# tokamak-network/Tokamak-zk-EVM

Hardware: AMD Instinct MI355X
Metric: constraints/sec (prove step) (higher is better)
Workload: dtype u32 limbs (255-bit Fr / 381-bit Fq modular integer arithmetic)

## Files before the change

include/tkmk.h:

```cpp
#ifndef TKMK_H
#define TKMK_H
#include <stdbool.h>
#include <stddef.h>
#include <stdint.h>

#ifdef __cplusplus
extern "C" {
#endif

typedef enum {
    TKMK_SUCCESS = 0,
    TKMK_ERR_INVALID_DEVICE = 1,
    TKMK_ERR_OUT_OF_MEMORY = 2,
    TKMK_ERR_INVALID_POINTER = 3,
    TKMK_ERR_ALLOCATION_FAILED = 4,
    TKMK_ERR_DEALLOCATION_FAILED = 5,
    TKMK_ERR_COPY_FAILED = 6,
    TKMK_ERR_SYNCHRONIZATION_FAILED = 7,
    TKMK_ERR_STREAM_CREATION_FAILED = 8,
    TKMK_ERR_STREAM_DESTRUCTION_FAILED = 9,
    TKMK_ERR_API_NOT_IMPLEMENTED = 10,
    TKMK_ERR_INVALID_ARGUMENT = 11,
    TKMK_ERR_NO_DEVICE = 12,
    TKMK_ERR_UNKNOWN = 999
// ... 270 lines not shown
tkmk_error bls12_381_polynomial_degree(const tkmk_polynomial *p, int64_t *degree);
tkmk_error bls12_381_polynomial_copy_coeffs(const tkmk_polynomial *p, size_t start, size_t count, tkmk_fr *out, bool out_on_device);
tkmk_error bls12_381_polynomial_get_coeff(const tkmk_polynomial *p, size_t idx, tkmk_fr *out_host);
tkmk_error bls12_381_polynomial_coeffs_device_ptr(tkmk_polynomial *p, tkmk_fr **ptr, size_t *n);
tkmk_error bls12_381_polynomial_evaluate(const tkmk_polynomial *p, const tkmk_fr *x_host, tkmk_fr *out_host);
tkmk_error bls12_381_polynomial_add(const tkmk_polynomial *a, const tkmk_polynomial *b, tkmk_polynomial **out);
tkmk_error bls12_381_polynomial_subtract(const tkmk_polynomial *a, const tkmk_polynomial *b, tkmk_polynomial **out);
tkmk_error bls12_381_polynomial_multiply(const tkmk_polynomial *a, const tkmk_polynomial *b, tkmk_polynomial **out);
tkmk_error bls12_381_polynomial_multiply_by_scalar(const tkmk_polynomial *a, const tkmk_fr *s_host, tkmk_polynomial **out);
tkmk_error bls12_381_polynomial_slice(const tkmk_polynomial *p, size_t offset, size_t stride, size_t size, tkmk_polynomial **out);
tkmk_error bls12_381_polynomial_divide(const tkmk_polynomial *num, const tkmk_polynomial *den, tkmk_polynomial **quot, tkmk_polynomial **rem);

tkmk_error tkmk_r1cs_eval_rows(const uint32_t *row_ptr_dev, const uint32_t *wire_dev, const tkmk_fr *coeff_dev, uint32_t n_rows,
                               uint32_t nnz, const tkmk_fr *variables_dev, uint32_t n_wires, uint32_t n_placements,
                               const uint32_t *out_slot_dev, uint32_t n, tkmk_fr *out_dev, tkmk_stream stream);

typedef struct tkmk_r1cs_library tkmk_r1cs_library;
tkmk_error tkmk_r1cs_library_create(uint32_t n_sub, const uint32_t *n_rows, const uint32_t *n_wires, const uint32_t *const *row_ptr,
                                    const uint32_t *const *wire, const tkmk_fr *const *coeff, tkmk_r1cs_library **out);
tkmk_error tkmk_r1cs_library_destroy(tkmk_r1cs_library *lib);
tkmk_error tkmk_r1cs_library_eval(const tkmk_r1cs_library *lib, const tkmk_fr *vars_dev, const uint32_t *placement_id_dev,
                                  const uint64_t *placement_var_offset_dev, uint32_t n_placements, uint32_t n, uint32_t s_max,
                                  tkmk_fr *u_dev, tkmk_fr *v_dev, tkmk_fr *w_dev, tkmk_stream stream);
tkmk_error tkmk_r1cs_library_mix(const tkmk_r1cs_library *lib, const tkmk_fr *const *weight_dev, const uint8_t *const *col_dev, uint32_t n,
                                 uint32_t n_cols, uint32_t out_stride, tkmk_fr *u_dev, tkmk_fr *v_dev, tkmk_fr *w_dev, tkmk_stream stream);
tkmk_error tkmk_fr_outer(const tkmk_fr *col_dev, uint32_t rows, const tkmk_fr *row_dev, uint32_t cols, uint32_t out_stride, tkmk_fr *out_dev,
                         tkmk_stream stream);
tkmk_error tkmk_witness_route(const tkmk_fr *vars_dev, const uint64_t *var_offset_dev, const uint32_t *slot_dev, uint32_t n_placements,
                              const uint32_t *list_wire_dev, const uint32_t *list_row_dev, uint32_t n_list, tkmk_fr *matrix_dev,
                              uint32_t matrix_stride, tkmk_fr *scalars_out_dev, uint32_t *index_out_dev, uint32_t index_inner,
                              int index_add_slot, tkmk_stream stream);
tkmk_error tkmk_fr_scatter_table(const tkmk_fr *table_dev, uint64_t table_len, const uint32_t *src_idx_dev, const uint32_t *dst_idx_dev,
                                 uint64_t n, tkmk_fr *out_dev, uint64_t out_len, tkmk_stream stream);
tkmk_error tkmk_witness_check_r1cs(const tkmk_fr *u_dev, const tkmk_fr *v_dev, const tkmk_fr *w_dev, uint32_t n_rows, uint32_t n_cols,
                                   uint32_t stride, uint32_t *bad_count_dev, uint32_t *first_bad_row_dev, uint64_t *total_bad_out,
                                   tkmk_stream stream);
tkmk_error tkmk_witness_check_copy(const tkmk_fr *b_dev, uint32_t rows, uint32_t cols, uint32_t stride, const uint32_t *dst_idx_dev,
                                   const uint32_t *src_x_dev, const uint32_t *src_y_dev, uint64_t n_entries, uint64_t *bad_entries_out,
                                   uint64_t *first_bad_entry_out, tkmk_stream stream);
tkmk_error tkmk_witness_check_copy_split(const tkmk_fr *b_local_dev, uint64_t local_cells, const uint32_t *dst_local_dev,
                                         const tkmk_fr *sources_dev, uint64_t n_sources, const uint32_t *src_slot_dev, uint64_t n,
                                         uint64_t *bad_entries_out, uint64_t *first_bad_entry_out, tkmk_stream stream);
tkmk_error tkmk_host_malloc(void **ptr, size_t bytes);
tkmk_error tkmk_host_free(void *ptr);

tkmk_error tkmk_msm_set_pipeline_streams(int n);
// ... 17 lines not shown
```

tokamak-zk-evm_amd/csrc/witness.hip:

```cpp
#include <mutex>
#include <vector>

#include "common.h"
#include "r1cs_library.h"

__global__ __launch_bounds__(256) void k_r1cs_library_eval(const uint32_t *__restrict__ rowptr, const uint32_t *__restrict__ wire,
                                                          const fr_t *__restrict__ coeff_mont, const uint32_t *__restrict__ desc,
                                                          const fr_t *__restrict__ vars, const uint32_t *__restrict__ pl_id,
                                                          const uint64_t *__restrict__ pl_off, uint32_t s_max, fr_t *__restrict__ u,
                                                          fr_t *__restrict__ v, fr_t *__restrict__ w) {
    const uint32_t p = blockIdx.z, m = blockIdx.y;
    const uint32_t row = blockIdx.x * blockDim.x + threadIdx.x;
    const uint32_t *d = desc + 8 * pl_id[p];
    if (row >= d[6]) return;
    const uint32_t *rp = rowptr + d[m];
    const uint32_t eb = d[3 + m];
    const fr_t *x = vars + pl_off[p];
    fr_t acc = Fr::zero();
    for (uint32_t k = rp[row]; k < rp[row + 1]; k++)
        acc = Fr::add(acc, Fr::mul(Fr::canon(tk_load(x + wire[eb + k])), tk_load(coeff_mont + eb + k)));
    fr_t *out = m == 0 ? u : m == 1 ? v : w;
    tk_store(out + (uint64_t)row * s_max + p, acc);
}
__global__ __launch_bounds__(256) void k_fr_to_mont(const fr_t *__restrict__ in, fr_t *__restrict__ out, uint64_t n) {
    uint64_t i = (uint64_t)blockIdx.x * blockDim.x + threadIdx.x;
    if (i < n) tk_store(out + i, Fr::to_mont(Fr::canon(tk_load(in + i))));
}

TK_API tkmk_error tkmk_r1cs_library_create(uint32_t n_sub, const uint32_t *n_rows, const uint32_t *n_wires, const uint32_t *const *row_ptr,
                                           const uint32_t *const *wire, const tkmk_fr *const *coeff, tkmk_r1cs_library **out) {
    if (!out || !n_rows || !n_wires || !row_ptr || !wire || !coeff) return TKMK_ERR_INVALID_POINTER;
    TK_TRY(tk_require_device());
    std::vector<uint32_t> rp_all, wire_all, desc(8 * (size_t)n_sub);
    std::vector<tkmk_fr> coeff_all;
// ... 38 lines not shown
    if (e == TKMK_SUCCESS) e = up((void **)&lib->d_coeff, coeff_all.data(), coeff_all.size() * sizeof(tkmk_fr));
    if (e == TKMK_SUCCESS) e = up((void **)&lib->d_desc, desc.data(), desc.size() * 4);
    if (e == TKMK_SUCCESS) {
        hipLaunchKernelGGL(k_fr_to_mont, tk_div_up(coeff_all.size(), 256), 256, 0, 0, (const fr_t *)lib->d_coeff, lib->d_coeff,
                           (uint64_t)coeff_all.size());
        if (hipGetLastError() != hipSuccess || hipDeviceSynchronize() != hipSuccess) e = TKMK_ERR_UNKNOWN;
    }
    if (e != TKMK_SUCCESS) {
        (void)hipFree(lib->d_rowptr), (void)hipFree(lib->d_wire), (void)hipFree(lib->d_coeff), (void)hipFree(lib->d_desc);
        delete lib;
        return e;
    }
    *out = lib;
    return TKMK_SUCCESS;
}
TK_API tkmk_error tkmk_r1cs_library_destroy(tkmk_r1cs_library *lib) {
    if (!lib) return TKMK_SUCCESS;
    (void)hipDeviceSynchronize();
    (void)hipFree(lib->d_rowptr), (void)hipFree(lib->d_wire), (void)hipFree(lib->d_coeff), (void)hipFree(lib->d_desc);
    delete lib;
    return TKMK_SUCCESS;
}

TK_API tkmk_error tkmk_r1cs_library_eval(const tkmk_r1cs_library *lib, const tkmk_fr *vars_dev, const uint32_t *placement_id_dev,
                                         const uint64_t *placement_var_offset_dev, uint32_t n_placements, uint32_t n, uint32_t s_max,
                                         tkmk_fr *u_dev, tkmk_fr *v_dev, tkmk_fr *w_dev, tkmk_stream stream) {
    if (!lib || !u_dev || !v_dev || !w_dev) return TKMK_ERR_INVALID_POINTER;
    if (n_placements && (!vars_dev || !placement_id_dev || !placement_var_offset_dev)) return TKMK_ERR_INVALID_POINTER;
    if (n_placements > s_max || lib->max_rows > n) return TKMK_ERR_INVALID_ARGUMENT;
    TK_TRY(tk_require_device());
    hipStream_t s = tk_stream(stream);
    const size_t bytes = (size_t)n * s_max * sizeof(fr_t);
    TK_HIP(hipMemsetAsync(u_dev, 0, bytes, s));
    TK_HIP(hipMemsetAsync(v_dev, 0, bytes, s));
    TK_HIP(hipMemsetAsync(w_dev, 0, bytes, s));
    if (n_placements && lib->max_rows) {
        hipLaunchKernelGGL(k_r1cs_library_eval, dim3(tk_div_up(lib->max_rows, 256), 3, n_placements), 256, 0, s, lib->d_rowptr, lib->d_wire,
                           (const fr_t *)lib->d_coeff, lib->d_desc, (const fr_t *)vars_dev, placement_id_dev, placement_var_offset_dev,
                           s_max, (fr_t *)u_dev, (fr_t *)v_dev, (fr_t *)w_dev);
        TK_HIP(hipGetLastError());
    }
    return TKMK_SUCCESS;
}

__global__ __launch_bounds__(256) void k_witness_route(const fr_t *__restrict__ vars, const uint64_t *__restrict__ var_off,
                                                      const uint32_t *__restrict__ slot, uint32_t n_placements,
                                                      const uint32_t *__restrict__ list_wire, const uint32_t *__restrict__ list_row,
                                                      uint32_t n_list, fr_t *__restrict__ matrix, uint32_t matrix_stride,
                                                      fr_t *__restrict__ scalars_out, uint32_t *__restrict__ index_out, uint32_t index_inner,
                                                      int index_add_slot) {
    uint64_t g = (uint64_t)blockIdx.x * blockDim.x + threadIdx.x;
    if (g >= (uint64_t)n_placements * n_list) return;
    uint32_t i = (uint32_t)(g / n_list), e = (uint32_t)(g - (uint64_t)i * n_list);
    fr_t val = tk_load(vars + var_off[i] + list_wire[e]);
    const uint32_t row = list_row[e], sl = slot[i];
    if (matrix) tk_store(matrix + (uint64_t)row * matrix_stride + sl, val);
    if (scalars_out) {
        tk_store(scalars_out + g, val);
        index_out[g] = row * index_inner + (index_add_slot ? sl : 0u);
    }
}
TK_API tkmk_error tkmk_witness_route(const tkmk_fr *vars_dev, const uint64_t *var_offset_dev, const uint32_t *slot_dev, uint32_t n_placements,
                                     const uint32_t *list_wire_dev, const uint32_t *list_row_dev, uint32_t n_list, tkmk_fr *matrix_dev,
                                     uint32_t matrix_stride, tkmk_fr *scalars_out_dev, uint32_t *index_out_dev, uint32_t index_inner,
                                     int index_add_slot, tkmk_stream stream) {
// ... 55 lines not shown
```

tokamak-zk-evm_amd/host/tkmk_fastparse.hpp:

```cpp
#pragma once
#include <fcntl.h>
#include <sched.h>
#include <sys/mman.h>
#include <sys/stat.h>
#include <unistd.h>

#if defined(__SSE2__)
#include <emmintrin.h>
#endif
#include <atomic>
#include <condition_variable>
#include <cstdlib>
#include <cstring>
#include <functional>
#include <mutex>
#include <string>
#include <thread>
#include <vector>

#include "tkmk_fr.hpp"

namespace tkmk {

inline unsigned host_threads() {
// ... 348 lines not shown
        while (i < n && is_ws(t[i])) i++;
        if (i < n && t[i] == ',') {
            i++;
            continue;
        }
        if (i < n && t[i] == ']') {
            i++;
            break;
        }
        fail("unexpected character", i);
    }
    count = cnt;
    return i;
}

}

struct WitnessLayout {
    std::vector<uint32_t> id;
    std::vector<uint64_t> off;
    uint64_t total = 0;
};

inline WitnessLayout parse_placement_variables_fast(const char *t, size_t n, const std::vector<uint32_t> &n_wires,
                                                    const std::function<ScalarField *(uint64_t)> &alloc, unsigned threads, uint32_t world = 1,
                                                    uint32_t rank = 0) {
    using namespace fastparse;
    const char *doc = "placementVariables.json";
    WitnessLayout L;
    std::vector<size_t> start = object_starts(t, n, threads);
    const size_t P = start.size();
    {
        Scanner s{t, 0, P ? start[0] : n, doc};
        s.expect('[');
        s.ws();
        if (P == 0) {
            Scanner e{t, s.i, n, doc};
            e.expect(']');
            e.ws();
            if (e.i != n) e.fail("trailing characters after the document");
            alloc(0);
            return L;
        }
        if (s.i != start[0]) s.fail("unexpected text before the first placement");
    }
    L.id.resize(P);
    std::atomic<size_t> next{0};
    parallel(threads, [&](unsigned) {
        for (;;) {
            size_t q0 = next.fetch_add(64);
            if (q0 >= P) break;
            for (size_t q = q0; q < q0 + 64 && q < P; q++) {
                size_t end = q + 1 < P ? start[q + 1] : n;
                Scanner s{t, start[q] + 1, end, doc};
                bool found = false;
                while (!found) {
                    size_t kb, ke;
                    s.str(kb, ke);
                    s.expect(':');
                    if (s.key_is(kb, ke, "subcircuitId")) {
                        uint64_t v = s.uint();
                        if (v >= n_wires.size()) throw Error("Invalid subcircuit id in placement_variables.");
                        L.id[q] = (uint32_t)v;
                        found = true;
                    } else if (s.peek('[')) {
                        const char *c = static_cast<const char *>(std::memchr(t + s.i, ']', end - s.i));
                        if (!c) s.fail("unterminated array");
                        s.i = (size_t)(c - t) + 1;
                    } else {
                        s.skip_scalar();
                    }
                    if (!found) {
                        if (s.peek(',')) s.i++;
                        else s.fail("placement without subcircuitId");
                    }
                }
            }
        }
    });
    L.off.resize(P);
    for (size_t q = 0; q < P; q++) {
        L.off[q] = L.total;
        if (q % world == rank) L.total += n_wires[L.id[q]];
    }
    ScalarField *vars = alloc(L.total);
    next = 0;
    parallel(threads, [&](unsigned) {
        for (;;) {
            size_t q = next.fetch_add(1);
            if (q >= P) break;
            if (q % world != rank) continue;
            size_t end = q + 1 < P ? start[q + 1] : n;
            Scanner s{t, start[q] + 1, end, doc};
            ScalarField *dst = vars + L.off[q];
            const uint32_t want = n_wires[L.id[q]];
            bool has_id = false, has_vars = false;
            for (;;) {
                size_t kb, ke;
                s.str(kb, ke);
                s.expect(':');
                if (s.key_is(kb, ke, "subcircuitId")) {
                    if (has_id) s.fail("duplicate key");
                    (void)s.uint();
                    has_id = true;
                } else if (s.key_is(kb, ke, "variables")) {
                    if (has_vars) s.fail("duplicate key");
                    s.expect('[');
                    uint32_t cnt = 0;
                    s.i = read_hex_array(t, s.i, end, dst, want, cnt, doc);
                    if (cnt != want) throw Error("Corrupted placement variables.");
                    has_vars = true;
                } else {
                    s.skip_scalar();
                }
                if (s.peek(',')) {
                    s.i++;
                    continue;
                }
                s.expect('}');
                break;
            }
            if (!has_id || !has_vars) s.fail("placement without subcircuitId / variables");
            s.between(q + 1 == P);
        }
    });
    return L;
}

struct PermutationColumns {
    std::vector<uint32_t> row, col, X, Y;
    size_t size() const { return row.size(); }
};
inline PermutationColumns parse_permutation_fast(const char *t, size_t n, unsigned threads) {
    using namespace fastparse;
    const char *doc = "permutation.json";
    PermutationColumns out;
    std::vector<size_t> start = object_starts(t, n, threads);
    const size_t P = start.size();
    {
        Scanner s{t, 0, P ? start[0] : n, doc};
        s.expect('[');
        s.ws();
        if (P == 0) {
            Scanner e{t, s.i, n, doc};
            e.expect(']');
            e.ws();
            if (e.i != n) e.fail("trailing characters after the document");
            return out;
// ... 49 lines not shown
```

tokamak-zk-evm_amd/host/tkmk_service.hpp:

```cpp
#pragma once
#include <sys/stat.h>

#include <fstream>
#include <future>

#include "tkmk_fastparse.hpp"
#include "tkmk_inputs.hpp"
#include "tkmk_prover.hpp"
#include "tkmk_witness_check.hpp"

namespace tkmk {



struct ProveTiming {
    double parse = 0, upload = 0, build = 0, binding = 0, init = 0;
    double prove[5] = {0, 0, 0, 0, 0};
    double write = 0, total = 0;
};

class ProverContext {
  public:
    SetupParams sp{};
    size_t m_i = 0;
// ... 270 lines not shown
        ProverContext &c;
        const Shard sh;
        const size_t lc;
        WitnessLayout W;
        std::vector<ScalarField> a_pub_user, a_pub_block, a_pub_function;
        witness_check::EffectivePermutation perm;
        std::vector<uint32_t> local_dst, local_x, local_y;
        std::vector<uint32_t> local_entry;
        DeviceVec<uint32_t> d_dst, d_x, d_y;
        size_t P = 0, PL = 0;
        std::vector<uint32_t> kind_first, slots, gslots, ids_local;
        std::vector<uint64_t> offs, offs_local;
        DeviceVec<ScalarField> d_vars;
        DeviceVec<uint32_t> d_id, d_slots, d_gslots;
        DeviceVec<uint64_t> d_off, d_offs;
        DeviceVec<ScalarField> u, v, w, b_ev, mid_sc, prv_sc, pub_sc;
        DeviceVec<uint32_t> mid_ix, prv_ix, pub_ix;
        uint64_t n_mid = 0, n_prv = 0, n_pub = 0;

        const std::vector<uint32_t> &dst() const { return sh.world > 1 ? local_dst : perm.dst; }
        const std::vector<uint32_t> &srcx() const { return sh.world > 1 ? local_x : perm.x; }
        const std::vector<uint32_t> &srcy() const { return sh.world > 1 ? local_y : perm.y; }

        WitnessLoader(ProverContext &ctx, const std::string &synth_dir, bool with_function) : c(ctx), sh(ctx.link ? ctx.link.shard : Shard{}), lc(sh.cols_of(ctx.sp.s_max)) {
            const size_t s_max = c.sp.s_max;
            {
                MappedFile perm_file(synth_dir + "/permutation.json");
                PermutationColumns cols = parse_permutation_fast(perm_file.data(), perm_file.size(), c.threads);
                host_trace("init: permutation.json parsed (%zu entries)", cols.size());
                start_reader(synth_dir, with_function);
                perm = witness_check::effective_permutation(cols, c.m_i, s_max);
            }
            if (sh.world > 1)
                for (size_t e = 0; e < perm.dst.size(); e++) {
                    const uint32_t row = perm.dst[e] / (uint32_t)s_max, col = perm.dst[e] % (uint32_t)s_max;
                    if (col % sh.world != sh.rank) continue;
                    local_dst.push_back(row * (uint32_t)lc + col / sh.world), local_x.push_back(perm.x[e]), local_y.push_back(perm.y[e]);
                    local_entry.push_back((uint32_t)e);
                }
        }
        void upload_permutation() {
            if (dst().empty()) return;
            d_dst = DeviceVec<uint32_t>::from_host(dst()), d_x = DeviceVec<uint32_t>::from_host(srcx()), d_y = DeviceVec<uint32_t>::from_host(srcy());
        }
        void join() {
            const size_t K = c.infos.size();
            std::string input_error;
            try {
                read_.get();
                host_trace("init: witness documents joined");
            } catch (const std::exception &e) {
                if (sh.world == 1) throw;
                input_error = e.what();
                if (input_error.empty()) input_error = "input error";
            }
            if (sh.world > 1) {
                const tkmk_error verdict = c.link.agree(c.link.comm, input_error.empty() ? TKMK_SUCCESS : TKMK_ERR_INVALID_ARGUMENT);
                if (!input_error.empty()) throw Error(input_error);
                if (verdict != TKMK_SUCCESS) throw Error("another rank of the sharded prover could not read its share of the synthesizer's documents");
            }
            P = W.id.size();
            std::vector<uint32_t> mine_q;
            for (size_t q = sh.rank; q < P; q += sh.world) mine_q.push_back((uint32_t)q);
            PL = mine_q.size();
            kind_first.assign(K + 1, 0), slots.assign(PL ? PL : 1, 0), gslots.assign(PL ? PL : 1, 0), ids_local.assign(PL ? PL : 1, 0);
            offs.assign(PL ? PL : 1, 0), offs_local.assign(PL ? PL : 1, 0);
            for (size_t k = 0; k < PL; k++) kind_first[W.id[mine_q[k]] + 1]++, ids_local[k] = W.id[mine_q[k]], offs_local[k] = W.off[mine_q[k]];
            for (size_t k = 0; k < K; k++) kind_first[k + 1] += kind_first[k];
            std::vector<uint32_t> cur(kind_first.begin(), kind_first.end() - 1);
            for (size_t k = 0; k < PL; k++) {
                const uint32_t q = mine_q[k];
                uint32_t at = cur[W.id[q]]++;
                slots[at] = (uint32_t)k, gslots[at] = q, offs[at] = W.off[q];
            }
        }
        void upload() {
            d_vars = DeviceVec<ScalarField>((size_t)W.total + 1);
            if (W.total) check(tkmk_memcpy_h2d(d_vars.ptr(), c.pinned_, (size_t)W.total * sizeof(ScalarField)), "witness upload");
            d_id = DeviceVec<uint32_t>::from_host(ids_local);
            d_off = DeviceVec<uint64_t>::from_host(offs_local);
            d_slots = DeviceVec<uint32_t>::from_host(slots), d_gslots = DeviceVec<uint32_t>::from_host(gslots);
            d_offs = DeviceVec<uint64_t>::from_host(offs);
        }
        void eval_uvw() {
            const size_t n = c.sp.n;
            u = DeviceVec<ScalarField>(n * lc), v = DeviceVec<ScalarField>(n * lc), w = DeviceVec<ScalarField>(n * lc);
            check(tkmk_r1cs_library_eval(c.lib_, d_vars.ptr(), d_id.ptr(), d_off.ptr(), (uint32_t)PL, (uint32_t)n, (uint32_t)lc, u.ptr(), v.ptr(), w.ptr(), nullptr),
                  "tkmk_r1cs_library_eval");
        }
        void route(bool binding_lists) {
            const size_t K = c.infos.size(), s_max = c.sp.s_max, m_i = c.m_i;
            const WireLists &iface_ = c.iface_, &prv_ = c.prv_, &pub_ = c.pub_;
            std::vector<uint64_t> mid_at(K), prv_at(K), pub_at(K);
            for (size_t k = 0; k < K; k++) {
                uint64_t cnt = kind_first[k + 1] - kind_first[k];
                mid_at[k] = n_mid, prv_at[k] = n_prv, pub_at[k] = n_pub;
                n_mid += cnt * iface_.count(k), n_prv += cnt * prv_.count(k), n_pub += cnt * pub_.count(k);
            }
            {
                std::vector<PlacementVariables> shape(P);
                uint64_t all_mid = 0, all_prv = 0;
                for (size_t q = 0; q < P; q++) shape[q].subcircuitId = W.id[q], all_mid += iface_.count(W.id[q]), all_prv += prv_.count(W.id[q]);
                if (all_mid != count_o_mid_nvar(shape, c.infos) || all_prv != count_o_prv_nvar(shape, c.infos)) throw Error("nVar mismatch while encoding statement");
            }
            if (n_mid >= (1ull << 31) || n_prv >= (1ull << 31)) throw Error("binding commitment too large");
            b_ev = DeviceVec<ScalarField>(m_i * lc);
            if (binding_lists) {
                mid_sc = DeviceVec<ScalarField>(n_mid + 1), prv_sc = DeviceVec<ScalarField>(n_prv + 1), pub_sc = DeviceVec<ScalarField>(n_pub + 1);
                mid_ix = DeviceVec<uint32_t>(n_mid + 1), prv_ix = DeviceVec<uint32_t>(n_prv + 1), pub_ix = DeviceVec<uint32_t>(n_pub + 1);
            }
            if (m_i * lc) check(tkmk_memset(b_ev.ptr(), 0, m_i * lc * sizeof(ScalarField)), "memset");
// ... 25 lines not shown
                      "tkmk_witness_route");
                check(tkmk_witness_route(d_vars.ptr(), vo, gsl, cnt, pub_.wire.ptr() + pub_.first[k], pub_.row.ptr() + pub_.first[k], pub_.count(k), nullptr, 0,
                                         pub_sc.ptr() + pub_at[k], pub_ix.ptr() + pub_at[k], 1, 0, nullptr),
                      "tkmk_witness_route");
            }
        }
        bool run_check(const ScalarField *u_dev, const ScalarField *v_dev, const ScalarField *w_dev, const ScalarField *b_dev, witness_check::Report &rep) const {
            witness_check::Inputs in;
            in.sp = &c.sp, in.infos = &c.infos, in.layout = &W, in.staged = c.pinned_;
            in.u = u_dev, in.v = v_dev, in.w = w_dev, in.b = b_dev;
            in.perm = &perm, in.d_dst = d_dst.ptr(), in.d_x = d_x.ptr(), in.d_y = d_y.ptr();
            in.a_pub_user = &a_pub_user, in.a_pub_block = &a_pub_block, in.a_pub_function = &a_pub_function;
            if (sh.world == 1) return witness_check::run(in, rep);
            witness_check::ShardInputs si;
            si.link = &c.link, si.lc = lc, si.placements = PL, si.local_entry = &local_entry, si.local_dst = &local_dst;
            return witness_check::run_sharded(in, si, rep);
        }

      private:
        void start_reader(const std::string &synth_dir, bool with_function) {
            read_ = staged_.get_future();
            reader_.t = std::thread([this, synth_dir, with_function] {
                std::unique_ptr<MappedFile> pv_file;
                try {
                    pv_file.reset(new MappedFile(synth_dir + "/placementVariables.json"));
                    W = parse_placement_variables_fast(pv_file->data(), pv_file->size(), c.n_wires_, [&](uint64_t total) { return c.staging(total); }, c.threads, sh.world, sh.rank);
                    host_trace("init: placementVariables.json parsed (%zu placements, %llu values kept)", W.id.size(), (unsigned long long)W.total);
                    if (W.id.size() > c.sp.s_max) throw Error("placement_variables length exceeds s_max.");
                    const json::Value jinst = json::read_file(synth_dir + "/instance.json");
                    a_pub_user = hex_list(jinst.at("a_pub_user"));
                    a_pub_block = hex_list(jinst.at("a_pub_block"));
                    if (with_function) a_pub_function = hex_list(jinst.at("a_pub_function"));
                    staged_.set_value();
                } catch (...) {
                    staged_.set_exception(std::current_exception());
                }
            });
        }
        std::promise<void> staged_;
        std::future<void> read_;
        struct Joined {
            std::thread t;
            ~Joined() { if (t.joinable()) t.join(); }
        } reader_;
    };

    static Error witness_refused(const witness_check::Report &rep) { return Error("the witness failed its check (TKMK_PROVER_CHECK_WITNESS): " + rep.reason); }

    bool check_witness(const std::string &synth_dir, witness_check::Report &rep) {
        if (link) throw Error("check_witness: not available on a sharded context (the copy section crosses columns: every rank calls check_witness_sharded instead)");
        return check_witness_steps(synth_dir, rep);
    }
    bool check_witness_sharded(const std::string &synth_dir, witness_check::Report &rep) {
        if (!link) return check_witness(synth_dir, rep);
        ShardSpan span(link);
        try {
            return check_witness_steps(synth_dir, rep);
        } catch (const Error &e) {
            const bool replicated_cause = e.code == TKMK_ERR_INVALID_ARGUMENT || e.code == TKMK_ERR_INVALID_POINTER;
            if (link.shard.world > 1 && !replicated_cause) (void)link.abort(link.comm);
            throw;
        } catch (...) {
            if (link.shard.world > 1) (void)link.abort(link.comm);
            throw;
        }
    }

// ... 1 lines not shown
    bool check_witness_steps(const std::string &synth_dir, witness_check::Report &rep) {
        const double t0 = Prover::now();
        WitnessLoader L(*this, synth_dir, true);
        L.upload_permutation();
        L.join();
        rep.parse_s = Prover::now() - t0;
        const double t1 = Prover::now();
        L.upload();
        rep.upload_s = Prover::now() - t1;
        const double t2 = Prover::now();
        L.eval_uvw();
        L.route(false);
        check(tkmk_device_synchronize(), "synchronize");
        rep.build_s = Prover::now() - t2;
        const double t3 = Prover::now();
        const bool ok = L.run_check(L.u.ptr(), L.v.ptr(), L.w.ptr(), L.b_ev.ptr(), rep);
        rep.check_s = Prover::now() - t3;
        rep.total_s = Prover::now() - t0;
        return ok;
    }

  public:

    std::pair<std::unique_ptr<Prover>, Binding> init(const std::string &synth_dir, const Mixer &mixer, ProveTiming &tm, CommitBatch::Pending *pending = nullptr) {
        using namespace prover_detail;
        const double t0 = Prover::now();
        const size_t n = sp.n, s_max = sp.s_max;
        host_trace("init: begin");
        const bool checked = witness_check::requested_at_prove();

        std::unique_ptr<Prover> p(new Prover());
        p->sp = sp, p->m_i = m_i, p->sigma = sigma.get(), p->mixer = mixer, p->lagrange = lagrange_;
        if (!link) {
            if (!commit_stream_) check(tkmk_stream_create(&commit_stream_), "stream_create");
            p->commit_stream = commit_stream_;
        }
        WitnessLoader L(*this, synth_dir, checked);
        {
            DeviceVec<ScalarField> e0 = s0_identity_.clone(), e1 = s1_identity_.clone();
            L.upload_permutation();
            if (!L.dst().empty()) {
                const size_t entries = L.dst().size();
                check(tkmk_fr_scatter_table(xp_.ptr(), xp_.len(), L.d_x.ptr(), L.d_dst.ptr(), entries, e0.ptr(), e0.len(), nullptr), "tkmk_fr_scatter_table");
                check(tkmk_fr_scatter_table(yp_.ptr(), yp_.len(), L.d_y.ptr(), L.d_dst.ptr(), entries, e1.ptr(), e1.len(), nullptr), "tkmk_fr_scatter_table");
            }
            p->s0XY = Poly::from_rou_evals_cols(e0, m_i, s_max), p->s1XY = Poly::from_rou_evals_cols(e1, m_i, s_max);
            p->s0_ev = std::move(e0), p->s1_ev = std::move(e1);
            p->s0_identity = &s0_identity_, p->s1_identity = &s1_identity_;
        }
        host_trace("init: s0 / s1 issued");
        L.join();
        tm.parse = Prover::now() - t0;

        const double t1 = Prover::now();
        L.upload();
        tm.upload = Prover::now() - t1;

        const double t2 = Prover::now();
        L.eval_uvw();
        p->uXY = Poly::from_rou_evals_cols(L.u, n, s_max), p->vXY = Poly::from_rou_evals_cols(L.v, n, s_max), p->wXY = Poly::from_rou_evals_cols(L.w, n, s_max);
// ... 123 lines not shown
```

tokamak-zk-evm_amd/tkmk/__init__.py:

```python
import ctypes
import os

import numpy as np

os.environ.setdefault("GPU_MAX_HW_QUEUES", "8")

_PKG = os.path.dirname(os.path.dirname(os.path.abspath(__file__)))
LIB_PATH = os.environ.get("TKMK_HIP_LIBRARY") or os.path.join(_PKG, "libtkmk_hip.so")
_lib = None


class TkmkError(RuntimeError):
    def __init__(self, code, where):
        self.code = code
        msg = lib().tkmk_error_string(code).decode() if _lib is not None else str(code)
        super().__init__("%s failed: %s (tkmk_error %d)" % (where, msg, code))


class Fr(ctypes.Structure):
    _fields_ = [("limbs", ctypes.c_uint32 * 8)]


class MSMConfig(ctypes.Structure):
    _fields_ = [
# ... 39 lines not shown
        ("is_result_on_device", ctypes.c_bool),
        ("is_async", ctypes.c_bool),
        ("batch_size", ctypes.c_int),
        ("columns_batch", ctypes.c_bool),
        ("ext", ctypes.c_void_p),
    ]


SYMBOLS = [
    "tkmk_device_count", "tkmk_set_device", "tkmk_get_available_memory", "tkmk_malloc", "tkmk_malloc_async", "tkmk_free",
    "tkmk_free_async", "tkmk_memcpy_h2d", "tkmk_memcpy_d2h", "tkmk_memcpy_d2d", "tkmk_memcpy_h2d_async",
    "tkmk_memcpy_d2h_async", "tkmk_memcpy_2d_d2d", "tkmk_memset", "tkmk_stream_create", "tkmk_stream_synchronize", "tkmk_stream_destroy", "tkmk_stream_set_background",
    "tkmk_device_synchronize", "tkmk_release_scratch", "tkmk_error_string", "tkmk_is_hip_build", "tkmk_keccak256", "tkmk_r1cs_index", "tkmk_msm_default_config", "bls12_381_msm", "bls12_381_g2_msm", "tkmk_g1_ntt", "tkmk_g1_ntt_axes", "tkmk_g1_prefix_sums", "tkmk_g1_scale", "bls12_381_msm_precompute_bases", "bls12_381_msm_precompute_bases_acc", "bn254_msm_precompute_bases", "tkmk_msm_multi", "bn254_msm", "tkmk_bn254_msm_multi", "bn254_get_root_of_unity", "bn254_ntt_init_domain", "bn254_ntt_release_domain",
    "bn254_ntt", "tkmk_bn254_bintt", "tkmk_bn254_fr_random_device",
    "tkmk_bn254_g1_batch_scalar_mul_device",
    "tkmk_ntt_default_config", "bls12_381_get_root_of_unity", "bls12_381_ntt_init_domain", "bls12_381_ntt_release_domain",
    "bls12_381_ntt", "tkmk_bintt", "tkmk_vecops_default_config", "bls12_381_vector_add", "bls12_381_vector_sub",
    "bls12_381_vector_mul", "bls12_381_vector_div", "bls12_381_vector_inv", "bls12_381_scalar_add_vec",
    "bls12_381_scalar_sub_vec", "bls12_381_scalar_mul_vec", "bls12_381_vector_sum", "bls12_381_vector_product",
    "bls12_381_matrix_transpose", "tkmk_vec_suffix_product", "tkmk_fr_random_device", "tkmk_gather_rows_device", "tkmk_g1_batch_scalar_mul_device", "tkmk_profile_enable",
    "tkmk_profile_reset", "tkmk_profile_get", "tkmk_diag_bench", "tkmk_diag_field_mul", "tkmk_diag_ffu", "tkmk_poly_find_degree",
    "tkmk_poly_place", "tkmk_poly_scale_coeffs", "tkmk_poly_mul_x_minus_one_evals", "tkmk_poly_mul_ones_x", "tkmk_poly_expr_eval", "tkmk_poly_expr_eval_views", "tkmk_poly_expr_eval_views_slab", "tkmk_poly_eval_x", "tkmk_poly_eval_y", "tkmk_poly_eval",
    "tkmk_poly_div_by_vanishing_opt", "tkmk_poly_div_by_ruffini", "tkmk_r1cs_eval_rows",
    "tkmk_msm_multi_ex", "tkmk_msm_segmented", "tkmk_msm_segmented_status", "bls12_381_msm_convert_bases", "tkmk_r1cs_library_create", "tkmk_r1cs_library_destroy", "tkmk_r1cs_library_eval",
    "tkmk_r1cs_library_mix", "tkmk_fr_outer",
    "tkmk_witness_route", "tkmk_fr_scatter_table", "tkmk_witness_check_r1cs", "tkmk_witness_check_copy", "tkmk_witness_check_copy_split", "tkmk_msm_set_pipeline_streams", "tkmk_msm_get_pipeline_streams", "tkmk_host_malloc", "tkmk_host_free", "tkmk_stats_reset", "tkmk_stats_get",
    "bls12_381_ntt_domain_size", "bn254_ntt_domain_size", "tkmk_poly_lincomb", "tkmk_bintt_padded", "tkmk_diag_device_switch", "tkmk_diag_gather_probe",
    "bls12_381_get_root_of_unity_with_generator", "tkmk_ntt_root_generator", "tkmk_ntt_set_root_generator", "tkmk_poly_geometric_grid", "tkmk_crs_identify_root", "tkmk_g1_check",
    "bls12_381_generate_random_affine_points", "bls12_381_generate_scalars", "bls12_381_polynomial_add", "bls12_381_polynomial_clone", "bls12_381_polynomial_coeffs_device_ptr", "bls12_381_polynomial_copy_coeffs", "bls12_381_polynomial_create_from_coefficients", "bls12_381_polynomial_create_from_rou_evaluations", "bls12_381_polynomial_degree", "bls12_381_polynomial_delete", "bls12_381_polynomial_divide", "bls12_381_polynomial_evaluate", "bls12_381_polynomial_get_coeff", "bls12_381_polynomial_multiply", "bls12_381_polynomial_multiply_by_scalar", "bls12_381_polynomial_nof_coeffs", "bls12_381_polynomial_slice", "bls12_381_polynomial_subtract", "bls12_381_vector_accumulate",
]


def lib():
    global _lib
    if _lib is None:
        if not os.path.exists(LIB_PATH):
            raise ImportError("libtkmk_hip.so is not built (run __graft_entry__.build()); there is no CPU fallback")
        _lib = ctypes.CDLL(LIB_PATH)
        _lib.tkmk_error_string.restype = ctypes.c_char_p
        _lib.tkmk_msm_default_config.restype = MSMConfig
        _lib.tkmk_ntt_default_config.restype = NTTConfig
        _lib.tkmk_vecops_default_config.restype = VecOpsConfig
    return _lib


def _check(code, where):
    if code != 0:
# ... 759 lines not shown
```

Before: 20.80 million.

## Stream witness parsing into sliced uploads and R1CS evaluation on a side stream

Splits placementVariables parsing into contiguous placement slices that become visible as parsing completes. A streamer thread uploads each finished slice and launches a ranged R1CS library eval on the commit stream, so H2D transfer and u/v/w evaluation overlap with JSON parsing. The remaining placements are handled after the join. The default is 8 slices, disabled in multi-device mode. It adds thread synchronisation complexity and reuses the commit stream, which could contend with other work.

```diff
diff --git a/include/tkmk.h b/include/tkmk.h
--- a/include/tkmk.h
+++ b/include/tkmk.h
@@ -316,6 +316,9 @@
 tkmk_error tkmk_r1cs_library_eval(const tkmk_r1cs_library *lib, const tkmk_fr *vars_dev, const uint32_t *placement_id_dev,
                                   const uint64_t *placement_var_offset_dev, uint32_t n_placements, uint32_t n, uint32_t s_max,
                                   tkmk_fr *u_dev, tkmk_fr *v_dev, tkmk_fr *w_dev, tkmk_stream stream);
+tkmk_error tkmk_r1cs_library_eval_range(const tkmk_r1cs_library *lib, const tkmk_fr *vars_dev, const uint32_t *placement_id_dev,
+                                        const uint64_t *placement_var_offset_dev, uint32_t first_placement, uint32_t n_placements, uint32_t n,
+                                        uint32_t s_max, tkmk_fr *u_dev, tkmk_fr *v_dev, tkmk_fr *w_dev, int zero_fill, tkmk_stream stream);
 tkmk_error tkmk_r1cs_library_mix(const tkmk_r1cs_library *lib, const tkmk_fr *const *weight_dev, const uint8_t *const *col_dev, uint32_t n,
                                  uint32_t n_cols, uint32_t out_stride, tkmk_fr *u_dev, tkmk_fr *v_dev, tkmk_fr *w_dev, tkmk_stream stream);
 tkmk_error tkmk_fr_outer(const tkmk_fr *col_dev, uint32_t rows, const tkmk_fr *row_dev, uint32_t cols, uint32_t out_stride, tkmk_fr *out_dev,
diff --git a/tokamak-zk-evm_amd/csrc/witness.hip b/tokamak-zk-evm_amd/csrc/witness.hip
--- a/tokamak-zk-evm_amd/csrc/witness.hip
+++ b/tokamak-zk-evm_amd/csrc/witness.hip
@@ -7,9 +7,9 @@
 __global__ __launch_bounds__(256) void k_r1cs_library_eval(const uint32_t *__restrict__ rowptr, const uint32_t *__restrict__ wire,
                                                           const fr_t *__restrict__ coeff_mont, const uint32_t *__restrict__ desc,
                                                           const fr_t *__restrict__ vars, const uint32_t *__restrict__ pl_id,
-                                                          const uint64_t *__restrict__ pl_off, uint32_t s_max, fr_t *__restrict__ u,
-                                                          fr_t *__restrict__ v, fr_t *__restrict__ w) {
-    const uint32_t p = blockIdx.z, m = blockIdx.y;
+                                                          const uint64_t *__restrict__ pl_off, uint32_t first, uint32_t s_max,
+                                                          fr_t *__restrict__ u, fr_t *__restrict__ v, fr_t *__restrict__ w) {
+    const uint32_t p = first + blockIdx.z, m = blockIdx.y;
     const uint32_t row = blockIdx.x * blockDim.x + threadIdx.x;
     const uint32_t *d = desc + 8 * pl_id[p];
     if (row >= d[6]) return;
@@ -94,25 +94,39 @@
     return TKMK_SUCCESS;
 }
 
+static tkmk_error r1cs_library_eval_range(const tkmk_r1cs_library *lib, const tkmk_fr *vars_dev, const uint32_t *placement_id_dev,
+                                          const uint64_t *placement_var_offset_dev, uint32_t first_placement, uint32_t n_placements, uint32_t n,
+                                          uint32_t s_max, tkmk_fr *u_dev, tkmk_fr *v_dev, tkmk_fr *w_dev, bool zero_fill, tkmk_stream stream) {
+    if (!lib || !u_dev || !v_dev || !w_dev) return TKMK_ERR_INVALID_POINTER;
+    if (n_placements && (!vars_dev || !placement_id_dev || !placement_var_offset_dev)) return TKMK_ERR_INVALID_POINTER;
+    if (first_placement > s_max || n_placements > s_max - first_placement || lib->max_rows > n) return TKMK_ERR_INVALID_ARGUMENT;
+    TK_TRY(tk_require_device());
+    hipStream_t s = tk_stream(stream);
+    if (zero_fill) {
+        const size_t bytes = (size_t)n * s_max * sizeof(fr_t);
+        TK_HIP(hipMemsetAsync(u_dev, 0, bytes, s));
+        TK_HIP(hipMemsetAsync(v_dev, 0, bytes, s));
+        TK_HIP(hipMemsetAsync(w_dev, 0, bytes, s));
+    }
+    if (n_placements && lib->max_rows) {
+        hipLaunchKernelGGL(k_r1cs_library_eval, dim3(tk_div_up(lib->max_rows, 256), 3, n_placements), 256, 0, s, lib->d_rowptr, lib->d_wire,
+                           (const fr_t *)lib->d_coeff, lib->d_desc, (const fr_t *)vars_dev, placement_id_dev, placement_var_offset_dev,
+                           first_placement, s_max, (fr_t *)u_dev, (fr_t *)v_dev, (fr_t *)w_dev);
+        TK_HIP(hipGetLastError());
+    }
+    return TKMK_SUCCESS;
+}
 TK_API tkmk_error tkmk_r1cs_library_eval(const tkmk_r1cs_library *lib, const tkmk_fr *vars_dev, const uint32_t *placement_id_dev,
                                          const uint64_t *placement_var_offset_dev, uint32_t n_placements, uint32_t n, uint32_t s_max,
                                          tkmk_fr *u_dev, tkmk_fr *v_dev, tkmk_fr *w_dev, tkmk_stream stream) {
-    if (!lib || !u_dev || !v_dev || !w_dev) return TKMK_ERR_INVALID_POINTER;
-    if (n_placements && (!vars_dev || !placement_id_dev || !placement_var_offset_dev)) return TKMK_ERR_INVALID_POINTER;
-    if (n_placements > s_max || lib->max_rows > n) return TKMK_ERR_INVALID_ARGUMENT;
-    TK_TRY(tk_require_device());
-    hipStream_t s = tk_stream(stream);
-    const size_t bytes = (size_t)n * s_max * sizeof(fr_t);
-    TK_HIP(hipMemsetAsync(u_dev, 0, bytes, s));
-    TK_HIP(hipMemsetAsync(v_dev, 0, bytes, s));
-    TK_HIP(hipMemsetAsync(w_dev, 0, bytes, s));
-    if (n_placements && lib->max_rows) {
-        hipLaunchKernelGGL(k_r1cs_library_eval, dim3(tk_div_up(lib->max_rows, 256), 3, n_placements), 256, 0, s, lib->d_rowptr, lib->d_wire,
-                           (const fr_t *)lib->d_coeff, lib->d_desc, (const fr_t *)vars_dev, placement_id_dev, placement_var_offset_dev,
-                           s_max, (fr_t *)u_dev, (fr_t *)v_dev, (fr_t *)w_dev);
-        TK_HIP(hipGetLastError());
-    }
-    return TKMK_SUCCESS;
+    return r1cs_library_eval_range(lib, vars_dev, placement_id_dev, placement_var_offset_dev, 0, n_placements, n, s_max, u_dev, v_dev, w_dev, true, stream);
+}
+TK_API tkmk_error tkmk_r1cs_library_eval_range(const tkmk_r1cs_library *lib, const tkmk_fr *vars_dev, const uint32_t *placement_id_dev,
+                                               const uint64_t *placement_var_offset_dev, uint32_t first_placement, uint32_t n_placements,
+                                               uint32_t n, uint32_t s_max, tkmk_fr *u_dev, tkmk_fr *v_dev, tkmk_fr *w_dev, int zero_fill,
+                                               tkmk_stream stream) {
+    return r1cs_library_eval_range(lib, vars_dev, placement_id_dev, placement_var_offset_dev, first_placement, n_placements, n, s_max, u_dev, v_dev, w_dev,
+                                   zero_fill != 0, stream);
 }
 
 __global__ __launch_bounds__(256) void k_witness_route(const fr_t *__restrict__ vars, const uint64_t *__restrict__ var_off,
diff --git a/tokamak-zk-evm_amd/host/tkmk_fastparse.hpp b/tokamak-zk-evm_amd/host/tkmk_fastparse.hpp
--- a/tokamak-zk-evm_amd/host/tkmk_fastparse.hpp
+++ b/tokamak-zk-evm_amd/host/tkmk_fastparse.hpp
@@ -394,12 +394,66 @@
     uint64_t total = 0;
 };
 
-inline WitnessLayout parse_placement_variables_fast(const char *t, size_t n, const std::vector<uint32_t> &n_wires,
-                                                    const std::function<ScalarField *(uint64_t)> &alloc, unsigned threads, uint32_t world = 1,
-                                                    uint32_t rank = 0) {
+class WitnessSlices {
+    mutable std::mutex mu_;
+    mutable std::condition_variable cv_;
+    std::vector<uint8_t> done_;
+    size_t P_ = 0, S_ = 0, prefix_ = 0, visible_ = 0;
+    ScalarField *staged_ = nullptr;
+    uint64_t total_ = 0;
+    bool begun_ = false, closed_ = false;
+    const size_t want_, max_placements_;
+
+  public:
+    explicit WitnessSlices(size_t want, size_t max_placements = SIZE_MAX) : want_(want ? want : 1), max_placements_(max_placements) {}
+    WitnessSlices(const WitnessSlices &) = delete;
+    WitnessSlices &operator=(const WitnessSlices &) = delete;
+
+    void begin(size_t placements, ScalarField *staged, uint64_t total) {
+        std::lock_guard<std::mutex> lk(mu_);
+        if (placements > max_placements_) return;
+        P_ = placements, S_ = want_ < placements ? want_ : placements, staged_ = staged, total_ = total;
+        done_.assign(P_, 0);
+        begun_ = true;
+        cv_.notify_all();
+    }
+    void placement_done(size_t q) {
+        std::lock_guard<std::mutex> lk(mu_);
+        if (!begun_) return;
+        done_[q] = 1;
+        while (prefix_ < P_ && done_[prefix_]) prefix_++;
+        size_t v = visible_;
+        while (v < S_ && first_of(v + 1) <= prefix_) v++;
+        if (v != visible_) visible_ = v, cv_.notify_all();
+    }
+    void close() {
+        std::lock_guard<std::mutex> lk(mu_);
+        closed_ = true;
+        cv_.notify_all();
+    }
+
+    bool layout(size_t &placements, ScalarField *&staged, uint64_t &total) const {
+        std::unique_lock<std::mutex> lk(mu_);
+        cv_.wait(lk, [&] { return begun_ || closed_; });
+        if (!begun_) return false;
+        placements = P_, staged = staged_, total = total_;
+        return true;
+    }
+    size_t wait(size_t have) const {
+        std::unique_lock<std::mutex> lk(mu_);
+        cv_.wait(lk, [&] { return visible_ > have || closed_; });
+        return visible_;
+    }
+    size_t slices() const { return S_; }
+    size_t first_of(size_t k) const { return S_ ? (P_ * k + S_ - 1) / S_ : 0; }
+};
+
+inline void parse_placement_variables_fast(const char *t, size_t n, const std::vector<uint32_t> &n_wires,
+                                           const std::function<ScalarField *(uint64_t)> &alloc, unsigned threads, WitnessLayout &L,
+                                           WitnessSlices *slices, uint32_t world = 1, uint32_t rank = 0) {
     using namespace fastparse;
     const char *doc = "placementVariables.json";
-    WitnessLayout L;
+    L = WitnessLayout{};
     std::vector<size_t> start = object_starts(t, n, threads);
     const size_t P = start.size();
     {
@@ -412,7 +466,7 @@
             e.ws();
             if (e.i != n) e.fail("trailing characters after the document");
             alloc(0);
-            return L;
+            return;
         }
         if (s.i != start[0]) s.fail("unexpected text before the first placement");
     }
@@ -456,12 +510,16 @@
         if (q % world == rank) L.total += n_wires[L.id[q]];
     }
     ScalarField *vars = alloc(L.total);
+    if (slices) slices->begin(P, vars, L.total);
     next = 0;
     parallel(threads, [&](unsigned) {
         for (;;) {
             size_t q = next.fetch_add(1);
             if (q >= P) break;
-            if (q % world != rank) continue;
+            if (q % world != rank) {
+                if (slices) slices->placement_done(q);
+                continue;
+            }
             size_t end = q + 1 < P ? start[q + 1] : n;
             Scanner s{t, start[q] + 1, end, doc};
             ScalarField *dst = vars + L.off[q];
@@ -494,8 +552,15 @@
             }
             if (!has_id || !has_vars) s.fail("placement without subcircuitId / variables");
             s.between(q + 1 == P);
+            if (slices) slices->placement_done(q);
         }
     });
+}
+inline WitnessLayout parse_placement_variables_fast(const char *t, size_t n, const std::vector<uint32_t> &n_wires,
+                                                    const std::function<ScalarField *(uint64_t)> &alloc, unsigned threads, uint32_t world = 1,
+                                                    uint32_t rank = 0) {
+    WitnessLayout L;
+    parse_placement_variables_fast(t, n, n_wires, alloc, threads, L, nullptr, world, rank);
     return L;
 }
 
diff --git a/tokamak-zk-evm_amd/host/tkmk_service.hpp b/tokamak-zk-evm_amd/host/tkmk_service.hpp
--- a/tokamak-zk-evm_amd/host/tkmk_service.hpp
+++ b/tokamak-zk-evm_amd/host/tkmk_service.hpp
@@ -316,13 +316,17 @@
         const std::vector<uint32_t> &srcx() const { return sh.world > 1 ? local_x : perm.x; }
         const std::vector<uint32_t> &srcy() const { return sh.world > 1 ? local_y : perm.y; }
 
-        WitnessLoader(ProverContext &ctx, const std::string &synth_dir, bool with_function) : c(ctx), sh(ctx.link ? ctx.link.shard : Shard{}), lc(sh.cols_of(ctx.sp.s_max)) {
+        WitnessLoader(ProverContext &ctx, const std::string &synth_dir, bool with_function, size_t slices = 1, tkmk_stream slice_stream = nullptr)
+            : c(ctx), sh(ctx.link ? ctx.link.shard : Shard{}), lc(sh.cols_of(ctx.sp.s_max)) {
             const size_t s_max = c.sp.s_max;
+            t_begin_ = Prover::now(), slice_stream_ = slice_stream;
+            if (slices > 1 && slice_stream && sh.world == 1) slices_.reset(new WitnessSlices(slices, s_max));
             {
                 MappedFile perm_file(synth_dir + "/permutation.json");
                 PermutationColumns cols = parse_permutation_fast(perm_file.data(), perm_file.size(), c.threads);
                 host_trace("init: permutation.json parsed (%zu entries)", cols.size());
                 start_reader(synth_dir, with_function);
+                if (slices_) start_streamer();
                 perm = witness_check::effective_permutation(cols, c.m_i, s_max);
             }
             if (sh.world > 1)
@@ -342,6 +346,11 @@
             std::string input_error;
             try {
                 read_.get();
+                if (streamer_.t.joinable()) {
+                    streamer_.t.join();
+                    if (stream_error_) std::rethrow_exception(stream_error_);
+                    check(tkmk_stream_synchronize(slice_stream_), "stream_synchronize");
+                }
                 host_trace("init: witness documents joined");
             } catch (const std::exception &e) {
                 if (sh.world == 1) throw;
@@ -369,18 +378,27 @@
             }
         }
         void upload() {
-            d_vars = DeviceVec<ScalarField>((size_t)W.total + 1);
-            if (W.total) check(tkmk_memcpy_h2d(d_vars.ptr(), c.pinned_, (size_t)W.total * sizeof(ScalarField)), "witness upload");
-            d_id = DeviceVec<uint32_t>::from_host(ids_local);
-            d_off = DeviceVec<uint64_t>::from_host(offs_local);
+            if (!preallocated_) d_vars = DeviceVec<ScalarField>((size_t)W.total + 1), d_id = DeviceVec<uint32_t>(ids_local.size()), d_off = DeviceVec<uint64_t>(offs_local.size());
+            const uint64_t v0 = streamed_ < PL ? offs_local[streamed_] : W.total;
+            if (W.total > v0) check(tkmk_memcpy_h2d(d_vars.ptr() + v0, c.pinned_ + v0, (size_t)(W.total - v0) * sizeof(ScalarField)), "witness upload");
+            if (indexed_ < ids_local.size()) {
+                check(tkmk_memcpy_h2d(d_id.ptr() + indexed_, ids_local.data() + indexed_, (ids_local.size() - indexed_) * sizeof(uint32_t)), "witness upload");
+                check(tkmk_memcpy_h2d(d_off.ptr() + indexed_, offs_local.data() + indexed_, (offs_local.size() - indexed_) * sizeof(uint64_t)), "witness upload");
+            }
             d_slots = DeviceVec<uint32_t>::from_host(slots), d_gslots = DeviceVec<uint32_t>::from_host(gslots);
             d_offs = DeviceVec<uint64_t>::from_host(offs);
         }
         void eval_uvw() {
             const size_t n = c.sp.n;
-            u = DeviceVec<ScalarField>(n * lc), v = DeviceVec<ScalarField>(n * lc), w = DeviceVec<ScalarField>(n * lc);
-            check(tkmk_r1cs_library_eval(c.lib_, d_vars.ptr(), d_id.ptr(), d_off.ptr(), (uint32_t)PL, (uint32_t)n, (uint32_t)lc, u.ptr(), v.ptr(), w.ptr(), nullptr),
-                  "tkmk_r1cs_library_eval");
+            if (!preallocated_) {
+                u = DeviceVec<ScalarField>(n * lc), v = DeviceVec<ScalarField>(n * lc), w = DeviceVec<ScalarField>(n * lc);
+                check(tkmk_r1cs_library_eval(c.lib_, d_vars.ptr(), d_id.ptr(), d_off.ptr(), (uint32_t)PL, (uint32_t)n, (uint32_t)lc, u.ptr(), v.ptr(), w.ptr(), nullptr),
+                      "tkmk_r1cs_library_eval");
+            } else if (streamed_ < PL) {
+                check(tkmk_r1cs_library_eval_range(c.lib_, d_vars.ptr(), d_id.ptr(), d_off.ptr(), (uint32_t)streamed_, (uint32_t)(PL - streamed_), (uint32_t)n, (uint32_t)lc,
+                                                   u.ptr(), v.ptr(), w.ptr(), streamed_ == 0, nullptr),
+                      "tkmk_r1cs_library_eval_range");
+            }
         }
         void route(bool binding_lists) {
             const size_t K = c.infos.size(), s_max = c.sp.s_max, m_i = c.m_i;
@@ -452,9 +470,17 @@
             read_ = staged_.get_future();
             reader_.t = std::thread([this, synth_dir, with_function] {
                 std::unique_ptr<MappedFile> pv_file;
+                struct Closer {
+                    WitnessSlices *s;
+                    ~Closer() { if (s) s->close(); }
+                };
                 try {
-                    pv_file.reset(new MappedFile(synth_dir + "/placementVariables.json"));
-                    W = parse_placement_variables_fast(pv_file->data(), pv_file->size(), c.n_wires_, [&](uint64_t total) { return c.staging(total); }, c.threads, sh.world, sh.rank);
+                    {
+                        Closer closer{slices_.get()};
+                        pv_file.reset(new MappedFile(synth_dir + "/placementVariables.json"));
+                        parse_placement_variables_fast(pv_file->data(), pv_file->size(), c.n_wires_, [&](uint64_t total) { return c.staging(total); }, c.threads, W, slices_.get(),
+                                                       sh.world, sh.rank);
+                    }
                     host_trace("init: placementVariables.json parsed (%zu placements, %llu values kept)", W.id.size(), (unsigned long long)W.total);
                     if (W.id.size() > c.sp.s_max) throw Error("placement_variables length exceeds s_max.");
                     const json::Value jinst = json::read_file(synth_dir + "/instance.json");
@@ -467,12 +493,55 @@
                 }
             });
         }
+        void stream_slices() {
+            size_t placements = 0;
+            ScalarField *staged = nullptr;
+            uint64_t total = 0;
+            if (!slices_->layout(placements, staged, total)) return;
+            const size_t n = c.sp.n;
+            tkmk_stream s = slice_stream_;
+            d_vars = DeviceVec<ScalarField>((size_t)total + 1);
+            d_id = DeviceVec<uint32_t>(placements), d_off = DeviceVec<uint64_t>(placements);
+            u = DeviceVec<ScalarField>(n * lc), v = DeviceVec<ScalarField>(n * lc), w = DeviceVec<ScalarField>(n * lc);
+            preallocated_ = true;
+            check(tkmk_memcpy_h2d_async(d_id.ptr(), W.id.data(), placements * sizeof(uint32_t), s), "witness upload");
+            check(tkmk_memcpy_h2d_async(d_off.ptr(), W.off.data(), placements * sizeof(uint64_t), s), "witness upload");
+            check(tkmk_stream_synchronize(s), "stream_synchronize");
+            indexed_ = placements;
+            for (size_t have = 0; have < slices_->slices(); have++) {
+                if (slices_->wait(have) <= have) break;
+                const size_t q0 = slices_->first_of(have), q1 = slices_->first_of(have + 1);
+                const uint64_t v0 = W.off[q0], v1 = q1 < placements ? W.off[q1] : total;
+                check(tkmk_memcpy_h2d_async(d_vars.ptr() + v0, staged + v0, (size_t)(v1 - v0) * sizeof(ScalarField), s), "witness upload");
+                check(tkmk_r1cs_library_eval_range(c.lib_, d_vars.ptr(), d_id.ptr(), d_off.ptr(), (uint32_t)q0, (uint32_t)(q1 - q0), (uint32_t)n, (uint32_t)lc, u.ptr(),
+                                                   v.ptr(), w.ptr(), have == 0, s),
+                      "tkmk_r1cs_library_eval_range");
+                streamed_ = q1;
+                host_trace("init: witness slice %zu of %zu issued (placements [%zu, %zu), %llu bytes, %.3f ms after init: begin)", have + 1, slices_->slices(), q0, q1,
+                           (unsigned long long)((v1 - v0) * sizeof(ScalarField)), 1e3 * (Prover::now() - t_begin_));
+            }
+        }
+        void start_streamer() {
+            streamer_.t = std::thread([this] {
+                try {
+                    stream_slices();
+                } catch (...) {
+                    stream_error_ = std::current_exception();
+                }
+            });
+        }
+        std::unique_ptr<WitnessSlices> slices_;
+        tkmk_stream slice_stream_ = nullptr;
+        std::exception_ptr stream_error_;
+        bool preallocated_ = false;
+        size_t streamed_ = 0, indexed_ = 0;
+        double t_begin_ = 0;
         std::promise<void> staged_;
         std::future<void> read_;
         struct Joined {
             std::thread t;
             ~Joined() { if (t.joinable()) t.join(); }
-        } reader_;
+        } reader_, streamer_;
     };
 
     static Error witness_refused(const witness_check::Report &rep) { return Error("the witness failed its check (TKMK_PROVER_CHECK_WITNESS): " + rep.reason); }
@@ -520,6 +589,12 @@
 
   public:
 
+    static size_t witness_slices() {
+        const char *e = getenv("TKMK_PROVER_WITNESS_SLICES");
+        const long v = e ? atol(e) : 8;
+        return v < 1 ? 1 : (size_t)v;
+    }
+
     std::pair<std::unique_ptr<Prover>, Binding> init(const std::string &synth_dir, const Mixer &mixer, ProveTiming &tm, CommitBatch::Pending *pending = nullptr) {
         using namespace prover_detail;
         const double t0 = Prover::now();
@@ -533,7 +608,7 @@
             if (!commit_stream_) check(tkmk_stream_create(&commit_stream_), "stream_create");
             p->commit_stream = commit_stream_;
         }
-        WitnessLoader L(*this, synth_dir, checked);
+        WitnessLoader L(*this, synth_dir, checked, link ? 1 : witness_slices(), commit_stream_);
         {
             DeviceVec<ScalarField> e0 = s0_identity_.clone(), e1 = s1_identity_.clone();
             L.upload_permutation();
diff --git a/tokamak-zk-evm_amd/tkmk/__init__.py b/tokamak-zk-evm_amd/tkmk/__init__.py
--- a/tokamak-zk-evm_amd/tkmk/__init__.py
+++ b/tokamak-zk-evm_amd/tkmk/__init__.py
@@ -85,7 +85,7 @@
     "tkmk_profile_reset", "tkmk_profile_get", "tkmk_diag_bench", "tkmk_diag_field_mul", "tkmk_diag_ffu", "tkmk_poly_find_degree",
     "tkmk_poly_place", "tkmk_poly_scale_coeffs", "tkmk_poly_mul_x_minus_one_evals", "tkmk_poly_mul_ones_x", "tkmk_poly_expr_eval", "tkmk_poly_expr_eval_views", "tkmk_poly_expr_eval_views_slab", "tkmk_poly_eval_x", "tkmk_poly_eval_y", "tkmk_poly_eval",
     "tkmk_poly_div_by_vanishing_opt", "tkmk_poly_div_by_ruffini", "tkmk_r1cs_eval_rows",
-    "tkmk_msm_multi_ex", "tkmk_msm_segmented", "tkmk_msm_segmented_status", "bls12_381_msm_convert_bases", "tkmk_r1cs_library_create", "tkmk_r1cs_library_destroy", "tkmk_r1cs_library_eval",
+    "tkmk_msm_multi_ex", "tkmk_msm_segmented", "tkmk_msm_segmented_status", "bls12_381_msm_convert_bases", "tkmk_r1cs_library_create", "tkmk_r1cs_library_destroy", "tkmk_r1cs_library_eval", "tkmk_r1cs_library_eval_range",
     "tkmk_r1cs_library_mix", "tkmk_fr_outer",
     "tkmk_witness_route", "tkmk_fr_scatter_table", "tkmk_witness_check_r1cs", "tkmk_witness_check_copy", "tkmk_witness_check_copy_split", "tkmk_msm_set_pipeline_streams", "tkmk_msm_get_pipeline_streams", "tkmk_host_malloc", "tkmk_host_free", "tkmk_stats_reset", "tkmk_stats_get",
     "bls12_381_ntt_domain_size", "bn254_ntt_domain_size", "tkmk_poly_lincomb", "tkmk_bintt_padded", "tkmk_diag_device_switch", "tkmk_diag_gather_probe",
```

Result: no change. 20.78 million (-0.1%).
